# ifpen/wfcrl-env

Hardware: AMD Instinct MI355X
Metric: farm_steps_per_sec (higher is better)
Workload: dtype f32

## Files before the change

include/wfstep.h:

```cpp
#ifndef WFSTEP_H
#define WFSTEP_H

#ifdef __cplusplus
extern "C" {
#endif

#define WF_ABI_VERSION 7

#define WF_OK 0
#define WF_E_INVALID -1
#define WF_E_UNSUPPORTED -2
#define WF_E_NODEVICE -3
#define WF_E_HIP -4
#define WF_E_NOMEM -5

#define WF_MAX_TURBINES 256
#define WF_MAX_TABLE 64
#define WF_MAX_TURBINE_TYPES 4

typedef struct wf_handle wf_handle;

typedef struct wf_model_params {
  double air_density, ambient_ti, shear, veer;
  double rotor_diameter, hub_height, tsr, pP, pT, gen_eff, ref_density;
// ... 40 lines not shown
int wf_set_layouts_counts(wf_handle* h, int n_layouts, const double* x, const double* y, const int* counts, const int* layout_of);

int wf_set_wind(wf_handle* h, const double* ws, const double* wd, int count, int on_device);

int wf_set_wind_counts(wf_handle* h, const double* ws, int n_ws, const double* wd, int n_wd, int on_device);

int wf_step(wf_handle* h, const float* yaw, float* power, float* wind_speed, float* wind_dir, float* load,
            int on_device);

int wf_sync(wf_handle* h);

#define WF_RISK_OVERLAP 1
#define WF_RISK_POWER_KNEE 2
#define WF_RISK_THRUST_RAMP 4
#define WF_RISK_THRUST_UNITY 8
#define WF_RISK_NEGATIVE_SPEED 16
int wf_set_risk_guard(wf_handle* h, double rel_band);
int wf_get_risk_flags(wf_handle* h, int* flags, int on_device);

int wf_set_risk_resolve(wf_handle* h, int mode);
int wf_get_risk_resolve(wf_handle* h, int* mode);
int wf_get_resolve_stats(wf_handle* h, int* n_resolved, int* raw_flags, int on_device);

typedef struct wf_env_params {
  float yaw_lo, yaw_hi, yaw_step;
  float actuator_rate;
  float dt;
  float budget;
  float load_coef;
  int discrete;
} wf_env_params;

int wf_env_config(wf_handle* h, const wf_env_params* p);

int wf_env_set_power_unit(wf_handle* h, int megawatts);

int wf_env_reset(wf_handle* h);

int wf_env_step(wf_handle* h, const float* action, float* reward, float* yaw, float* power, float* wind_speed,
                float* wind_dir, float* load, int on_device);

int wf_env_set_prev_wind(wf_handle* h, const double* wind_speed , int on_device);

int wf_env_state(wf_handle* h, float* yaw, float* acc, int* moves, int set, int on_device);

typedef struct wf_wind_dist {
// ... 49 lines not shown
```

wfcrl-env_amd/_lib.py:

```python
from __future__ import annotations

import ctypes as C
import os
import subprocess
from pathlib import Path

PKG_DIR = Path(__file__).resolve().parent
LIB_PATH = PKG_DIR / "libwfstep.so"

WF_OK = 0
WF_RISK_OVERLAP = 1
WF_RISK_POWER_KNEE = 2
WF_RISK_THRUST_RAMP = 4
WF_RISK_THRUST_UNITY = 8
WF_RISK_NEGATIVE_SPEED = 16
WF_E = {-1: "WF_E_INVALID", -2: "WF_E_UNSUPPORTED", -3: "WF_E_NODEVICE", -4: "WF_E_HIP", -5: "WF_E_NOMEM"}

_MODEL_DOUBLES = (
    "air_density", "ambient_ti", "shear", "veer",
    "rotor_diameter", "hub_height", "tsr", "pP", "pT", "gen_eff", "ref_density",
    "alpha", "beta", "ka", "kb", "ad", "bd", "dm",
    "ch_initial", "ch_constant", "ch_ai", "ch_downstream",
    "eps_gain", "num_eps", "kappa", "gch_gain", "overlap_thresh", "near_wake_c",
    "defl_alpha", "defl_beta", "defl_ka", "defl_kb",
# ... 46 lines not shown
    "wf_turbine_table": (C.c_int, [C.c_char_p, C.POINTER(C.c_int), C.POINTER(C.POINTER(C.c_double)),
                                   C.POINTER(C.POINTER(C.c_double)), C.POINTER(C.POINTER(C.c_double))]),
    "wf_create": (C.c_int, [C.c_int, C.POINTER(_P)]),
    "wf_destroy": (C.c_int, [_P]),
    "wf_set_stream": (C.c_int, [_P, _P, C.c_int]),
    "wf_get_stream": (_P, [_P]),
    "wf_set_model": (C.c_int, [_P, C.POINTER(ModelParams)]),
    "wf_set_turbine_types": (C.c_int, [_P, C.c_int, C.POINTER(TurbineDef), C.POINTER(C.c_int)]),
    "wf_get_turbine_types": (C.c_int, [_P, C.POINTER(C.c_int)]),
    "wf_set_layout": (C.c_int, [_P, C.c_int, _P, _P]),
    "wf_set_batch": (C.c_int, [_P, C.c_int]),
    "wf_set_layouts": (C.c_int, [_P, C.c_int, _P, _P, _P]),
    "wf_set_layouts_counts": (C.c_int, [_P, C.c_int, _P, _P, _P, _P]),
    "wf_set_wind": (C.c_int, [_P, _P, _P, C.c_int, C.c_int]),
    "wf_set_wind_counts": (C.c_int, [_P, _P, C.c_int, _P, C.c_int, C.c_int]),
    "wf_wind_sample_binned": (C.c_int, [_P, C.c_ulonglong, C.POINTER(WindDist), C.c_double]),
    "wf_step": (C.c_int, [_P, _P, _P, _P, _P, _P, C.c_int]),
    "wf_sync": (C.c_int, [_P]),
    "wf_set_risk_guard": (C.c_int, [_P, C.c_double]),
    "wf_get_risk_flags": (C.c_int, [_P, _P, C.c_int]),
    "wf_set_risk_resolve": (C.c_int, [_P, C.c_int]),
    "wf_get_risk_resolve": (C.c_int, [_P, C.POINTER(C.c_int)]),
    "wf_get_resolve_stats": (C.c_int, [_P, C.POINTER(C.c_int), _P, C.c_int]),
    "wf_wind_sample": (C.c_int, [_P, C.c_ulonglong, C.POINTER(WindDist)]),
    "wf_wind_series": (C.c_int, [_P, C.c_int, _P, _P, _P, C.c_ulonglong]),
    "wf_wind_series_step": (C.c_int, [_P]),
    "wf_get_wind": (C.c_int, [_P, _P, _P, C.c_int]),
    "wf_env_config": (C.c_int, [_P, C.POINTER(EnvParams)]),
    "wf_env_set_power_unit": (C.c_int, [_P, C.c_int]),
    "wf_env_reset": (C.c_int, [_P]),
    "wf_env_state": (C.c_int, [_P, _P, _P, _P, C.c_int, C.c_int]),
    "wf_env_set_prev_wind": (C.c_int, [_P, _P, C.c_int]),
    "wf_env_step": (C.c_int, [_P, _P, _P, _P, _P, _P, _P, _P, C.c_int]),
    "wf_timing_begin": (C.c_int, [_P]),
    "wf_timing_end": (C.c_int, [_P, C.POINTER(C.c_float)]),
    "wf_get_kernel_info": (C.c_int, [_P, C.POINTER(KernelInfo)]),
    "wf_set_kernel_choice": (C.c_int, [_P, C.POINTER(KernelChoice)]),
    "wf_get_kernel_choice": (C.c_int, [_P, C.POINTER(KernelChoice)]),
    "wf_get_calibration": (C.c_int, [_P, C.POINTER(C.c_int), C.POINTER(C.c_float)]),
    "wf_get_fly_calibration": (C.c_int, [_P, C.POINTER(C.c_int), C.POINTER(C.c_float)]),
    "wf_get_mixed_launch": (C.c_int, [_P, C.POINTER(C.c_int), C.POINTER(C.c_float)]),
    "wf_calibrate": (C.c_int, [_P]),
    "wf_set_calibration": (C.c_int, [_P, C.c_int, C.c_int]),
    "wf_last_error": (C.c_char_p, [_P]),
}

# ... 50 lines not shown
```

wfcrl-env_amd/backend.py:

```python
from __future__ import annotations

import ctypes as C

import numpy as np

from . import _lib
from ._lib import EnvParams, KernelChoice, KernelInfo, ModelParams, WindDist, check


def _is_torch(a) -> bool:
    return type(a).__module__.startswith("torch")


def default_model() -> dict:
    p = ModelParams()
    check(_lib.load().wf_default_model(C.byref(p)))
    d = {n: getattr(p, n) for n in _lib._MODEL_DOUBLES}
    d.update({n: bool(getattr(p, n)) for n in _lib._MODEL_SWITCHES})
    n = p.n_table
    d["table_ws"] = [p.table_ws[i] for i in range(n)]
    d["table_ct"] = [p.table_ct[i] for i in range(n)]
    d["table_cp"] = [p.table_cp[i] for i in range(n)]
    return d

# ... 301 lines not shown
                    out[k] = torch.empty(shapes[k], device=dev, dtype=torch.float32)
            ptrs = [out[k].data_ptr() if k in want else None for k in order]
            check(self._lib.wf_env_step(self._h, action.data_ptr() if action is not None else None, *ptrs, 1), self._h)
            return {k: out[k] for k in want}
        if action is not None:
            action = np.ascontiguousarray(action, dtype=np.float32).reshape(B, N)
        out = dict(out or {})
        for k in want:
            if k not in out:
                out[k] = np.empty(shapes[k], np.float32)
        ptrs = [out[k].ctypes.data if k in want else None for k in order]
        check(self._lib.wf_env_step(self._h, action.ctypes.data if action is not None else None, *ptrs, 0), self._h)
        return {k: out[k] for k in want}

    def sync(self):
        check(self._lib.wf_sync(self._h), self._h)

    def set_risk_guard(self, rel_band: float):
        check(self._lib.wf_set_risk_guard(self._h, float(rel_band)), self._h)

    def set_risk_resolve(self, mode: int | bool = 1):
        check(self._lib.wf_set_risk_resolve(self._h, int(mode)), self._h)

    def risk_resolve(self) -> int:
        m = C.c_int(0)
        check(self._lib.wf_get_risk_resolve(self._h, C.byref(m)), self._h)
        return int(m.value)

    def resolve_stats(self) -> dict:
        if not self.risk_resolve():
            raise RuntimeError("resolve_stats() needs the float64 re-solve on (set_risk_resolve(1), the default); with it off "
                               "the flags of the last step are risk_flags()")
        n = C.c_int(0)
        raw = np.empty(self.env_batch, np.int32)
        check(self._lib.wf_get_resolve_stats(self._h, C.byref(n), raw.ctypes.data, 0), self._h)
        return {"n_resolved": int(n.value), "raw_flags": raw}

    def risk_flags(self, as_torch: bool = False):
        B = self.env_batch
        if as_torch:
            import torch

            self._follow_torch_stream()
            f = torch.empty(B, dtype=torch.int32, device=f"cuda:{self.device_id}")
            check(self._lib.wf_get_risk_flags(self._h, f.data_ptr(), 1), self._h)
            return f
# ... 90 lines not shown
```

wfcrl-env_amd/csrc/wf_abi.hip:

```cpp
#include "wf_handle.h"

namespace wfi {

thread_local std::string g_create_error;

void free_batch(wf_handle* h) {
  hipFree(h->d_ws); hipFree(h->d_wd); hipFree(h->d_gx); hipFree(h->d_gy); hipFree(h->d_gidx); hipFree(h->d_flags);
  hipFree(h->d_farm_tie);
  hipFree(h->d_dir_perm); hipFree(h->d_sort_keys); hipFree(h->d_sort_vals); hipFree(h->d_sort_tmp);
  h->d_dir_perm = h->d_sort_vals = nullptr; h->d_sort_keys = nullptr; h->d_sort_tmp = nullptr;
  h->sort_tmp_bytes = h->dir_perm_cap = 0; h->dir_slots = 0;
  hipFree(h->d_res_list); hipFree(h->d_res_count); hipFree(h->d_flags_raw);
  h->d_res_list = h->d_res_count = h->d_flags_raw = nullptr;
  if (h->h_res_seen) (void)hipHostFree(h->h_res_seen);
  h->h_res_seen = nullptr;
  h->d_flags = h->d_farm_tie = nullptr;
  hipFree(h->d_yaw); hipFree(h->d_out);
  hipFree(h->d_env_yaw); hipFree(h->d_env_acc); hipFree(h->d_env_act); hipFree(h->d_env_out); hipFree(h->d_env_moves);
  if (h->h_env_act) hipHostFree(h->h_env_act);
  if (h->h_env_out) hipHostFree(h->h_env_out);
  h->d_env_yaw = h->d_env_acc = h->d_env_act = h->d_env_out = h->h_env_act = h->h_env_out = nullptr;
  h->d_env_moves = nullptr;
  hipFree(h->d_series_ws); hipFree(h->d_series_wd); hipFree(h->d_series_start); hipFree(h->d_ws_prev);
  hipFree(h->d_pair_tab); hipFree(h->d_pair_first); h->d_pair_tab = nullptr; h->d_pair_first = nullptr; h->pair_dirty = true;
// ... 257 lines not shown
  if (wspd) std::memcpy(wspd, h->h_out + bn, sizeof(float) * bn);
  if (wdir) std::memcpy(wdir, h->h_out + 2 * bn, sizeof(float) * bn);
  if (load) std::memcpy(load, h->h_out + 3 * bn, sizeof(float) * bn * 4);
  return WF_OK;
}
int wf_set_risk_guard(wf_handle* h, double rel_band) {
  if (!h) return WF_E_INVALID;
  if (!(rel_band >= 0.0) || !(rel_band < 0.5)) return fail(h, WF_E_INVALID, "risk guard band must be in [0, 0.5)");
  h->guard_rel = rel_band;
  h->guard_user = true;
  h->consts.guard_inv = rel_band > 0.0 ? (float)(1.0 / rel_band) : 1125899906842624.0f;
  return WF_OK;
}

int wf_set_risk_resolve(wf_handle* h, int mode) {
  if (!h) return WF_E_INVALID;
  if (mode < 0 || mode > 2) return fail(h, WF_E_INVALID, "risk resolve mode must be 0 (off), 1 (flagged farms) or 2 (every farm)");
  if (!h->types.empty() && mode == 0)
    return fail(h, WF_E_INVALID, "several turbine definitions (wf_set_turbine_types): the float32 kernels know one table, mode 0 cannot be served");
  h->resolve_mode = mode;
  return WF_OK;
}

int wf_get_risk_resolve(wf_handle* h, int* mode) {
  if (!h || !mode) return WF_E_INVALID;
  *mode = h->types.empty() ? h->resolve_mode : 2;
  return WF_OK;
}

int wf_get_resolve_stats(wf_handle* h, int* n_resolved, int* raw_flags, int on_device) {
  if (!h) return WF_E_INVALID;
  if (h->B <= 0) return fail(h, WF_E_INVALID, "wf_set_batch must be called first");
  WF_ON_DEVICE(h);
  if (!h->d_res_list || !h->res_last) {
    if (n_resolved) *n_resolved = 0;
    if (raw_flags) return wf_get_risk_flags(h, raw_flags, on_device);
    return WF_OK;
  }
  if (raw_flags)
    WF_HIP(h, hipMemcpyAsync(raw_flags, h->d_flags_raw, sizeof(int) * h->B, on_device ? hipMemcpyDeviceToDevice : hipMemcpyDeviceToHost,
                             h->stream));
  if (n_resolved) WF_HIP(h, hipMemcpyAsync(n_resolved, h->d_res_count + h->res_parity, sizeof(int), hipMemcpyDeviceToHost, h->stream));
  if (n_resolved || (raw_flags && !on_device)) WF_HIP(h, hipStreamSynchronize(h->stream));
  return WF_OK;
}

// ... 36 lines not shown
```

wfcrl-env_amd/csrc/wf_device.h:

```cpp
#pragma once

#define WF_TABLE_PAD 64
#define WF_BUCKETS 2048

struct WfConsts {
  int N;
  float D, invD;
  float off[3];
  float yoff[3];
  float shearf[3];
  float uinf_f;
  float decay_a[3];
  float exp_c;
  float zc[7], zc2[7], ez[7];
  float inv_eps2, m_half_inv_eps4, yl2_small;
  float zm[7], zm2[7], ezm[7];
  int mirror_core_n;
  float gam_top, gam_bot;
  float gam_wr;
  float ks_top, ks_bot, ks_core;
  float alpha4, beta2, ka, kb, ad, bd, dm03;
  float alpha4_d, beta2_d, ka_d, kb_d;
  float sw_steer, sw_tv;
  float e0c1, e0c2;
  float sz0v;
  float near_c;
  float kdef;
  float kdef_sy0v;
  float far_k;
  int far_on;
  float ch_c, ch_ai, ch_down;
  float amb, amb2, gch_gain, overlap_thr, twoD;
  float rho, pw, dens_f;
  int n_table;
  float bucket_h_inv, bucket_x0;
  int max_probe;
  double fifteenD_d;
  double q_d;
  float ct_kappa;
  float guard_inv, inv_overlap_thr, knee_kappa;
  int veer_on;
  float cos_veer;
  float veer_c2, veer_s2;
  float veer_bq;
};

struct WfTables {
  float knot[WF_TABLE_PAD];
  float ct[WF_TABLE_PAD];
  float ct_slope[WF_TABLE_PAD];
  float pw[WF_TABLE_PAD];
  float pw_slope[WF_TABLE_PAD];
  unsigned char bucket[WF_BUCKETS];
// ... 78 lines not shown
```

wfcrl-env_amd/csrc/wf_handle.h:

```cpp
#pragma once
#include <hip/hip_runtime.h>

#include <cmath>
#include <cstdio>
#include <cstdlib>
#include <cstring>
#include <mutex>
#include <new>
#include <string>
#include <vector>

#include "../../include/wfstep.h"
#include "wf_device.h"
#include "wf_resolve.h"

extern "C" hipError_t wfk_launch_resolve(const WfResolveConsts* c, const WfResolveArgs* a, int B, int all, int* raw_flags,
                                         int n_cu, hipStream_t s);
extern "C" int wfk_num_variants();
extern "C" void wfk_variant(int i, int* G, int* S, const void** fn);
extern "C" int wfk_variant_has_table(int i);
extern "C" int wfk_tab_waves();
extern "C" const void* wfk_variant_fn(int i, int kind);
extern "C" hipError_t wfk_launch_geometry(int n_env, int N, const double* lx, const double* ly, const double* centre,
                                          int layout_mode, const int* layout_of, const int* layout_n, const double* wd, int wd_stride, double* gx,
// ... 104 lines not shown
  int* d_ll_flag = nullptr;
  float* d_src_log = nullptr;
  size_t ll_groups_cap = 0, log_records_cap = 0;
  int* d_farm_tie = nullptr;
  int* d_dir_perm = nullptr;
  float* d_sort_keys = nullptr;
  int* d_sort_vals = nullptr;
  void* d_sort_tmp = nullptr;
  size_t sort_tmp_bytes = 0, dir_perm_cap = 0;
  int dir_slots = 0;
  int geo_tie_block = 0;
  int farm_ties = 2;
  bool wind_sync = true;
  int ll_ties = 2;
  wf_kernel_choice choice{0, 0, -1, 0, 0, -1, -1, -1, -1, -1};
  int n_cu = 256;
  bool calib_done = false;
  int calib_code = -1;
  int mix_main = 0;
  bool tab_slot = false;
  float calib_ms[8] = {};
  int fly_calib = 0;
  float fly_calib_ms[2] = {};
  int resolve_mode = 1;
  WfResolveConsts rconsts{};
  double* d_tab64 = nullptr;
  int *d_res_list = nullptr, *d_res_count = nullptr, *d_flags_raw = nullptr;
  int* h_res_seen = nullptr;
  int res_parity = 0;
  bool res_last = false;
  int res_mask = 0;
  struct TurbineType {
    std::vector<double> ws, ct, cp;
    double tsr, pP, gen_eff, ref_density;
  };
  std::vector<TurbineType> types;
  std::vector<int> type_of;
  double* d_tab64_mt = nullptr;
  double* d_type_consts = nullptr;
  int* d_type_of = nullptr;
};

namespace wfi {

extern thread_local std::string g_create_error;

// ... 58 lines not shown
```

wfcrl-env_amd/csrc/wf_kernels_ll.hip:

```cpp
#include <hip/hip_runtime.h>

#include <cstring>
#include <type_traits>
#include <utility>

#include "wf_kernel_common.h"

namespace {

template <class F, int... I>
__device__ __forceinline__ void static_for_impl(F&& f, std::integer_sequence<int, I...>) {
  (f(std::integral_constant<int, I>{}), ...);
}
template <int N, class F>
__device__ __forceinline__ void static_for(F&& f) {
  static_for_impl(f, std::make_integer_sequence<int, N>{});
}

__device__ __forceinline__ void sincos_yaw(float x, float& s, float& c) {
  const float x2 = x * x;
  s = x * fmaf(x2, fmaf(x2, fmaf(x2, fmaf(x2, 2.7557319e-6f, -1.9841270e-4f), 8.3333333e-3f), -1.6666667e-1f), 1.0f);
  c = fmaf(x2, fmaf(x2, fmaf(x2, fmaf(x2, fmaf(x2, -2.7557319e-7f, 2.4801587e-5f), -1.3888889e-3f), 4.1666667e-2f), -0.5f), 1.0f);
  if (__any(fabsf(x) > 0.8f)) {
    float s2, c2;
// ... 440 lines not shown
    const float ti = fabsf(R.ch_pref) * tipow;
    const float tia = in15 ? ti * (cnt * (1.0f / 9.0f)) : 0.0f;
    const float cand = fsqrt(fmaf(tia, tia, c.amb2));
#pragma unroll
    for (int j = 0; j < 3; ++j) {
      const float cm = (bits & (1 << j)) ? cand : 0.0f;
      TI[p][j] = __uint_as_float(max(__float_as_uint(TI[p][j]), __float_as_uint(cm)));
    }
  };

  float psum = 0.0f, lsum = 0.0f;
  const int n_real = ga.n_real ? ga.n_real[env] : N;
#ifdef WF_LL_STAMP
  unsigned long long st_acc[12] = {0, 0, 0, 0, 0, 0, 0, 0, 0, 0, 0, 0};
  WF_T(st_begin);
#endif
  int q = 0;
  const size_t wave_rec0 = (size_t)(slot - eiw) * n_pad;
  float2* const log_hot = reinterpret_cast<float2*>(src_log + wave_rec0 * WF_LOG_HOT_FLOATS);
  float4* const log_cold = reinterpret_cast<float4*>(src_log + log_cold_offset + wave_rec0 * WF_LOG_COLD_FLOATS) + eiw;
  float4* const bndL = reinterpret_cast<float4*>(yaw_lds) + (size_t)wave * n_pad;
  constexpr int HOT_INSTR = (CH / 2) * EPW * 16 >= 1024 ? (CH / 2) * EPW * 16 / 1024 : 1;
  constexpr int HOT_F4 = HOT_INSTR * 64;
  float4* const hotL = reinterpret_cast<float4*>(yaw_lds) + (size_t)WPB * n_pad + (size_t)wave * (2 * HOT_F4);
  auto stage_hot = [&](int qq, int i_first) {
    const char* g0 = reinterpret_cast<const char*>(reinterpret_cast<const float4*>(log_hot) + (size_t)(i_first >> 1) * EPW);
    char* l0 = reinterpret_cast<char*>(hotL + (qq & 1) * HOT_F4);
#pragma unroll
    for (int ch = 0; ch < HOT_INSTR; ++ch) lds_dma16(g0 + ch * 1024 + lane * 16, l0 + ch * 1024, true);
  };
  auto hot_index = [&](int i) { return 2 * ((size_t)(i >> 1) * EPW + eiw) + (i & 1); };
  auto load_hot = [&](int i) { return log_hot[hot_index(i)]; };
  auto load_cold = [&](int i) {
    const float4* lp = log_cold + (size_t)i * (3 * EPW);
    ColdRec r;
    r.a = lp[0]; r.b = lp[EPW]; r.c = lp[2 * EPW];
    return r;
  };
  const float snw_f = c.near_c * 0.70710678118f;
  auto unpack = [&](const float2 h, const ColdRec& r) {
    SrcLog R;
    R.Gy = h.x * h.y; R.Gwt = h.y;
    R.sy0d = r.a.x; R.sz0d = r.a.y; R.sM = r.a.z; R.tan_th0 = r.a.w;
    R.sy0v = r.b.x; R.x0d = r.b.y; R.kyd = r.b.z; R.pj = r.b.w;
    R.x0v = r.c.x; R.kyv = r.c.y; R.ch_pref = r.c.z; R.ix0v = r.c.w;
    R.snw = snw_f * R.sM;
    R.kdef = (R.sM * R.sM) * (R.sy0v * c.kdef_sy0v);
// ... 42 lines not shown
    const int n_src = min(N, first_own + GS);
    const int n_chunks = (n_src + CH - 1) / CH;
    float2 hot_nx = make_float2(0.0f, 0.0f);
    ColdRec cold_nx = {};
    double xs_nx = 0.0, ys_nx = 0.0;
    if (first_own > 0) {
      if constexpr (!TAB) {
        hot_nx = load_hot(0);
        cold_nx = load_cold(0);
        xs_nx = gx[gofs];
        ys_nx = gy[gofs];
      }
    }

    auto fly_record = [&](auto PP, double xi, double yi) {
      constexpr int p = decltype(PP)::value;
      constexpr int q = TAB ? 0 : p;
      float4 r;
      r.x = (float)(xt_d[q] - xi);
      r.y = (float)(yt_d[q] - yi);
      r.z = (xt_d[q] <= xi + c.fifteenD_d) ? 1.0f : 0.0f;
      r.w = __int_as_float((xt_d[q] > xi + 0.1) ? 8 : 0);
      return r;
    };

    auto own_source = [&](auto PS, int i, const float* recs) {
      constexpr int ps = decltype(PS)::value;
      const int src = gbase + ((i - first_own) - ps * G);
      __builtin_amdgcn_s_setprio(3);
      WF_T(so_0);
      float vsum = 0.0f;
#pragma unroll
      for (int k2 = 0; k2 < 9; ++k2) vsum += V[ps][k2];
      const float m3 = __shfl(cube_sum(esq[ps]), src);
      const float Vmean = __shfl(vsum, src) * (1.0f / 9.0f);
      float TIs[3];
#pragma unroll
      for (int j = 0; j < 3; ++j) TIs[j] = __shfl(TI[ps][j], src);
      const float yaw_i = __shfl(yaw_t[ps], src);
      const float cg = __shfl(cg_t[ps], src), sg = __shfl(sg_t[ps], src);
      WF_T(so_1);
      WF_ACC(6, so_0, so_1);
      SrcLog Sc;
      const float ubar = fcbrt_pos(m3 * (1.0f / 9.0f));
      unsigned trisk;
      const float ct = table_ct(c, T, ubar, trisk) * cg;
// ... 79 lines not shown
      if (lane == src) {
#pragma unroll
        for (int j = 0; j < 3; ++j) TI[ps][j] = fmaxf(TI[ps][j] + X.dTI, amb0);
      }
      Sc.sy0v = c.sz0v * cg;
      if constexpr (VEER) Sc.sy0v *= c.cos_veer;
      Sc.snw = c.near_c * fsqrt(0.5f * ct);
      Sc.kdef = ct * cg * c.kdef;
      Sc.ch_pref = c.ch_c * fexp2(c.ch_ai * flog2(a));
      const float x0num_v = c.D * cg * (1.0f + s_c) * (1.0f / 1.41421356237f);
      const float b2om = c.beta2 * om_sc, b2om_d = c.beta2_d * om_sc;
      Sc.x0d = x0num_d * frcp(fmaf(c.alpha4_d, TIs[0], b2om_d));
      Sc.kyd = fmaf(c.ka_d, TIs[0], c.kb_d);
      Sc.pj = pfac * frcp(Sc.kyd);
      Sc.x0v = x0num_v * frcp(fmaf(c.alpha4, TIs[0] + X.dTI, b2om));
      Sc.kyv = fmaf(c.ka, TIs[0] + X.dTI, c.kb);
      X.TI0 = TIs[0]; X.TI1 = TIs[1]; X.TI2 = TIs[2];
      const bool split = !((TIs[0] == TIs[1]) && (TIs[1] == TIs[2]));
      Sc.ch_pref = split ? -Sc.ch_pref : Sc.ch_pref;
      Sc.ix0v = frcp(Sc.x0v);
      Sc.inv_s0d = frcp(Sc.sy0d * Sc.sz0d);
      Sc.d0 = Sc.tan_th0 * Sc.x0d;
      if (J + 1 < nblk) {
        if (sub == 0) {
          log_hot[hot_index(i)] = make_float2(Sc.Gwt != 0.0f ? Sc.Gy * frcp(Sc.Gwt) : 0.0f, Sc.Gwt);
          float4* lp = log_cold + (size_t)i * (3 * EPW);
          lp[0] = make_float4(Sc.sy0d, Sc.sz0d, Sc.sM, Sc.tan_th0);
          lp[EPW] = make_float4(Sc.sy0v, Sc.x0d, Sc.kyd, Sc.pj);
          lp[2 * EPW] = make_float4(Sc.x0v, Sc.kyv, Sc.ch_pref, Sc.ix0v);
          if (split) *reinterpret_cast<float4*>(logx + (size_t)i * WF_LOG_SIDE_FLOATS) = make_float4(X.TI0, X.TI1, X.TI2, X.dTI);
        }
        const float s0 = VEER ? c.sz0v : Sc.sy0v;
        float kyv_m = Sc.kyv, bb = fmaf(-Sc.kyv, Sc.x0v, s0);
        float db = fabsf(Sc.tan_th0 * Sc.x0d) + 2.2f * fabsf(Sc.pj);
        if (__any(split)) {
          const float TImax = fmaxf(TIs[0], fmaxf(TIs[1], TIs[2])), TImin = fminf(TIs[0], fminf(TIs[1], TIs[2]));
          const float x0d_m = x0num_d * frcp(fmaf(c.alpha4_d, TImin, b2om_d));
          const float pj_m = pfac * frcp(fmaf(c.ka_d, TImin, c.kb_d));
          kyv_m = fmaf(c.ka, TImax + X.dTI, c.kb);
          bb = split ? s0 : bb;
          db = fabsf(Sc.tan_th0 * x0d_m) + 2.2f * fabsf(pj_m);
        }
        const float dbo = db + c.off[2];
        float k6 = c.far_k * kyv_m, b6 = fmaf(c.far_k, bb, dbo), n6 = fmaf(c.far_k, fmaxf(Sc.snw, s0), dbo);
        k6 = wave_max<G>(k6);
        b6 = wave_max<G>(b6);
        n6 = wave_max<G>(n6);
        if (!c.far_on) { k6 = 0.0f; b6 = 0.0f; n6 = 3.0e38f; }
        if (lane == 0) bndL[i] = make_float4(k6, b6, n6, 0.0f);
      }
      WF_T(so_4);
      WF_ACC(9, so_3, so_4);
      const float xs_[4] = {X.TI0, X.TI1, X.TI2, X.dTI};
      static_for<S>([&](auto PP) {
        constexpr int p = decltype(PP)::value;
        if constexpr (p == ps) pass2(PP, Sc, xs_, false, ex[p], ex[p].x > 0.0f, yt_d[TAB ? 0 : p], yi_d);
        else if constexpr (p > ps) pass2(PP, Sc, xs_, false, ex[p], tvalid[p], yt_d[TAB ? 0 : p], yi_d);
      });
      WF_T(so_5);
      WF_ACC(10, so_4, so_5);
      __builtin_amdgcn_s_setprio(0);
    };

    for (int cq = 0; cq < n_chunks; ++cq, ++q) {
      if constexpr (TAB) {
        if (cq == 0 && first_own > 0) wf_dma_wait();
        if (cq + 1 < n_chunks || J + 1 < nblk) stage_chunk(q + 1);
        if (cq + 1 < n_chunks && (cq + 1) * CH < first_own) stage_hot(q + 1, (cq + 1) * CH);
      }
      const float* buf = &prow[q & 1][0];
      const int i0 = cq * CH;
      const int k_log = min(max(first_own - i0, 0), CH);
      const int k_end = min(n_src - i0, CH);
      WF_T(st_a);
      auto within_bound = [&](const float4 bnd, float dx, float dy) {
        return fabsf(dy) < fmaxf(fmaf(bnd.x, dx, bnd.y), bnd.z) + fabsf(fmaf(c.bd, dx, c.ad));
      };
      if constexpr (TAB) {
        if (k_log > 0) {
          unsigned long long near_bits, pair_bits;
          {
            const int kk = lane / GS, rr = lane % GS;
            const float2 e = *reinterpret_cast<const float2*>(buf + (kk * GS + rr) * WF_PAIR_STRIDE + WF_PAIR_DX);
            const float4 bnd = bndL[min(i0 + kk, n_pad - 1)];
            pair_bits = __ballot(kk < k_log && (J * GS + rr) < N && within_bound(bnd, e.x, e.y));
            near_bits = pair_bits;
#pragma unroll
            for (int sh = 1; sh < GS; sh <<= 1) near_bits |= near_bits >> sh;
            unsigned long long rep = 0ull;
#pragma unroll
            for (int kq = 0; kq < CH; ++kq) rep |= 1ull << (kq * GS);
            near_bits &= rep;
          }
          ColdRec cold_nx = {};
          if (near_bits) cold_nx = load_cold(i0 + (__builtin_ctzll(near_bits) / GS));
          static_assert(GS % 2 == 0 && CH % 2 == 0, "logged sources come in pairs");
#pragma unroll 1
          for (int k = 0; k < k_log; k += 2) {
            const float4 hot2 = hotL[(q & 1) * HOT_F4 + (k >> 1) * EPW + eiw];
            float4 cf[S][9];
// ... 57 lines not shown
          hot_nx = load_hot(inx);
          cold_nx = load_cold(inx);
          xs_nx = gx[gofs + inx];
          ys_nx = gy[gofs + inx];
          const float4 bnd = bndL[i];
          float4 exr[S];
          int nr = 0;
          static_for<S>([&](auto PP) {
            constexpr int p = decltype(PP)::value;
            exr[p] = fly_record(PP, xs_d, ys_d);
            nr |= (int)tvalid[p] & (int)within_bound(bnd, exr[p].x, exr[p].y);
          });
          const bool near = __any(nr != 0);
          const SrcLog Sl = unpack(hot, cold);
          static_for<S>([&](auto PP) {
            constexpr int p = decltype(PP)::value;
            if (tvalid[p]) apply_fly(PP, exr[p].x, exr[p].y, hot.x * hot.y, hot.y);
            if (near) pass2(PP, Sl, side, true, exr[p], tvalid[p], yt_d[TAB ? 0 : p], ys_d);
          });
        }
      }
      WF_T(st_b);
      WF_ACC(0, st_a, st_b);
#pragma unroll 1
      for (int k = k_log; k < k_end; ++k) {
        const int i = i0 + k;
        const float* recs = buf + (k * GS) * WF_PAIR_STRIDE;
        const int slot_of_source = (i - first_own) / G;
        static_for<S>([&](auto PS) {
          if (slot_of_source == decltype(PS)::value) own_source(PS, i, recs);
        });
      }
      WF_T(st_c);
      WF_ACC(1, st_b, st_c);
      if constexpr (TAB) {
        wf_dma_wait();
        __syncthreads();
      }
      WF_T(st_d);
      WF_ACC(2, st_c, st_d);
    }
    if constexpr (TAB) {
      if (J + 1 < nblk) stage_hot(q, 0);
    }
    WF_T(st_e);

#pragma unroll
    for (int p = 0; p < S; ++p) {
// ... 98 lines not shown
      const float r = psum * invN * 1.0e-3f * frcp(wr * wr * wr) - ea.load_coef * lsum * invN * 0.25f;
      ea.reward[env] = r;
    }
  }
}

constexpr int kLLWaves = 4;

template <int G, int S, bool TAB, bool MC1, bool VEER = false>
static hipError_t launch_ll(const WfConsts* c, const WfTables* tab, const int* gidx, const double* ws, const double* wd,
                            int wind_stride, const float* yaw, float* power, float* o_ws, float* o_wd, float* load, int B,
                            const WfEnvArgs* env, const float* ll_tab, const int* cross_tie, float* src_log, size_t log_records,
                            const WfGroupArgs* grp, const double* gx, const double* gy, hipStream_t s) {
  constexpr int fpb = kLLWaves * (64 / G);
  WfGroupArgs ga = *grp;
  const int n_farms = ga.env_end ? ga.env_end - ga.env_base : B;
  const int grid = ga.blk_group ? (ga.n_slots + fpb - 1) / fpb : (n_farms + fpb - 1) / fpb;
  WfConsts cc = *c;
  WfEnvArgs ea;
  if (env) ea = *env; else memset(&ea, 0, sizeof(ea));
  size_t group_floats = wfk_ll_table_floats(cc.N, G * S);
  int n_pad = ((cc.N + G * S - 1) / (G * S)) * (G * S);
  constexpr int hot_bytes = 32768 / (G * G * S) >= 1024 ? 32768 / (G * G * S) : 1024;
  const size_t dyn_lds = sizeof(float4) * (size_t)kLLWaves * n_pad + (TAB ? (size_t)kLLWaves * 2 * hot_bytes : 0);
  size_t log_cold_offset = log_records * WF_LOG_HOT_FLOATS, log_side_offset = log_records * WF_LOG_FLOATS;
  void* args[] = {&cc, &tab, &gidx, &ws, &wd, &wind_stride, &yaw, &power, &o_ws, &o_wd, &load, &B, &ea, &ll_tab,
                  &group_floats, &cross_tie, &src_log, &log_cold_offset, &log_side_offset, &n_pad, &ga, &gx, &gy};
  const void* fn = (const void*)&wf_step_ll_kernel<G, S, false, TAB, MC1, kLLWaves, VEER>;
  if constexpr (TAB) {
    if (wind_stride == 0) fn = (const void*)&wf_step_ll_kernel<G, S, true, TAB, MC1, kLLWaves, VEER>;
  }
  if constexpr (S == 1 && (MC1 || !TAB) && !VEER) {
    static int n_cu_of[64] = {};
    int dev = 0, n_cu = 0;
    if (hipGetDevice(&dev) == hipSuccess && dev >= 0 && dev < 64) {
      n_cu = n_cu_of[dev];
      if (n_cu == 0 && hipDeviceGetAttribute(&n_cu, hipDeviceAttributeMultiprocessorCount, dev) == hipSuccess) n_cu_of[dev] = n_cu;
    }
    if (n_cu > 0 && grid <= 2 * n_cu)
      fn = wind_stride == 0 ? (const void*)&wf_step_ll_kernel<G, S, true, TAB, MC1, kLLWaves, VEER, true>
                            : (const void*)&wf_step_ll_kernel<G, S, false, TAB, MC1, kLLWaves, VEER, true>;
  }
  return hipLaunchKernel(fn, dim3(grid), dim3(64 * kLLWaves), args, dyn_lds, s);
}

extern "C" int wfk_ll_farms_per_block(int G) { return kLLWaves * (64 / G); }
#ifdef WF_LL_STAMP
// ... 98 lines not shown
```

wfcrl-env_amd/csrc/wf_model.hip:

```cpp
#include "wf_handle.h"

namespace {

const double kCtFrom3[45] = {
    0.99,       0.99,       0.97373036, 0.92826162, 0.89210543, 0.86100905, 0.835423,   0.81237673, 0.79225789,
    0.77584769, 0.7629228,  0.76156073, 0.76261984, 0.76169723, 0.75232027, 0.74026851, 0.72987175, 0.70701647,
    0.54054532, 0.45509459, 0.39343381, 0.34250785, 0.30487242, 0.27164979, 0.24361964, 0.21973831, 0.19918151,
    0.18131868, 0.16537679, 0.15103727, 0.13998636, 0.1289037,  0.11970413, 0.11087113, 0.10339901, 0.09617888,
    0.09009926, 0.08395078, 0.0791188,  0.07448356, 0.07050731, 0.06684119, 0.06345518, 0.06032267, 0.05741999};
const double kCpFrom3SurveyA5[45] = {
    0.1780851,  0.28907459, 0.34902166, 0.3847278,  0.40605878, 0.4202279,  0.42882274, 0.43387274, 0.43622267,
    0.43684468, 0.43657497, 0.43651053, 0.4365612,  0.43651728, 0.43590309, 0.43467276, 0.43322955, 0.43003137,
    0.37655587, 0.33328466, 0.29700574, 0.26420779, 0.23839379, 0.21459275, 0.19382354, 0.1756635,  0.15970926,
    0.14561785, 0.13287856, 0.12130194, 0.11219941, 0.10311631, 0.09545392, 0.08813781, 0.08186763, 0.07585005,
    0.07071926, 0.06557558, 0.06148104, 0.05755207, 0.05413366, 0.05097969, 0.04806545, 0.04536883, 0.04287006};
const double kCpFrom3Floris3[45] = {
    0.178085, 0.289075, 0.349022, 0.384728, 0.406059, 0.420228, 0.428823, 0.433873, 0.436223,
    0.436845, 0.436575, 0.436511, 0.436561, 0.436517, 0.435903, 0.434673, 0.433230, 0.430466,
    0.378869, 0.335199, 0.297991, 0.266092, 0.238588, 0.214748, 0.193981, 0.175808, 0.159835,
    0.145741, 0.133256, 0.122157, 0.112257, 0.103399, 0.095449, 0.088294, 0.081836, 0.075993,
    0.070692, 0.065875, 0.061484, 0.057476, 0.053809, 0.050447, 0.047358, 0.044518, 0.041900,
};
double g_tab_ws[51], g_tab_ct[51], g_tab_cp[51], g_tab_cp_a5[51];
std::once_flag g_tab_once;
// ... 74 lines not shown
  c.gam_bot = (float)(inv2pi * (M_PI / 8.0) * D * vel_bot * uinf);
  c.gam_wr = (float)(inv2pi * 0.25 * 2.0 * M_PI * D / m.tsr);
  c.alpha4 = (float)(4.0 * m.alpha); c.beta2 = (float)(2.0 * m.beta);
  c.ka = (float)m.ka; c.kb = (float)m.kb; c.ad = (float)m.ad; c.bd = (float)m.bd; c.dm03 = (float)(0.3 * m.dm);
  c.alpha4_d = (float)(4.0 * m.defl_alpha); c.beta2_d = (float)(2.0 * m.defl_beta);
  c.ka_d = (float)m.defl_ka; c.kb_d = (float)m.defl_kb;
  c.sw_steer = m.enable_secondary_steering ? 2.0f : 0.0f;
  c.sw_tv = m.enable_transverse_velocities ? 1.0f : 0.0f;
  c.e0c1 = (float)(3.0 * std::exp(1.0 / 12.0)); c.e0c2 = (float)(3.0 * std::exp(1.0 / 3.0));
  c.sz0v = (float)(D / (2.0 * std::sqrt(2.0)));
  c.near_c = (float)(m.near_wake_c * D);
  c.kdef = (float)(D * D / 8.0);
  c.ch_c = (float)(m.ch_constant * std::pow(m.ambient_ti, m.ch_initial));
  c.ch_ai = (float)m.ch_ai; c.ch_down = (float)m.ch_downstream;
  c.amb = (float)m.ambient_ti; c.amb2 = (float)(m.ambient_ti * m.ambient_ti);
  c.gch_gain = m.enable_yaw_added_recovery ? (float)m.gch_gain : 0.0f; c.overlap_thr = (float)m.overlap_thresh;
  c.twoD = (float)(2.0 * D); c.fifteenD_d = 15.0 * D;
  c.q_d = D / 4.0;
  c.guard_inv = h->guard_rel > 0.0 ? (float)(1.0 / h->guard_rel) : 1125899906842624.0f;
  c.inv_overlap_thr = (float)(1.0 / m.overlap_thresh);
  c.far_on = (h->choice.far_skip != 0 && m.ka >= 0.0 && m.kb >= 0.0 && m.defl_ka >= 0.0 && m.defl_kb >= 0.0 && m.alpha >= 0.0 &&
              m.beta >= 0.0 && m.defl_alpha >= 0.0 && m.defl_beta >= 0.0) ? 1 : 0;
  c.far_k = c.far_on ? 6.12f : 1.0e30f;
  c.ct_kappa = 5.0f;
  c.knee_kappa = 30.0f;
  {
    const double vr = m.veer * M_PI / 180.0;
    c.veer_on = m.veer != 0.0 ? 1 : 0;
    c.cos_veer = (float)std::cos(vr);
    c.veer_c2 = (float)(std::cos(vr) * std::cos(vr)); c.veer_s2 = (float)(std::sin(vr) * std::sin(vr));
    c.veer_bq = (float)(std::sin(2.0 * vr) * D / 4.0);
    c.kdef_sy0v = (float)((D * D / 8.0) / ((D / (2.0 * std::sqrt(2.0))) * std::cos(vr)));
  }
  c.rho = (float)m.ref_density; c.pw = (float)(m.pP / 3.0);
  c.dens_f = (float)std::cbrt(m.air_density / m.ref_density);

  WfTables t;
  const double area = M_PI * R * R;
  std::vector<double> pwv(n);
  for (int i = 0; i < n; ++i) pwv[i] = 0.5 * area * h->tcp[i] * m.gen_eff * h->tws[i] * h->tws[i] * h->tws[i];
  for (int i = 0; i < WF_TABLE_PAD; ++i) {
    const bool in = i < n;
    t.knot[i] = in ? (float)h->tws[i] : 3.0e38f;
    t.ct[i] = in ? (float)h->tct[i] : 0.f;
    t.pw[i] = in ? (float)pwv[i] : 0.f;
    const bool seg = i + 1 < n;
// ... 233 lines not shown
```

Measured before the change: 81.92 million.

## Solve independent wake sources as a parallel level with snapshot rollback

Adds a speculative 'level' path to the low-latency kernel: all owned sources in a chunk are processed together, with one parallel velocity accumulation and parameter computation, instead of the sequential per-source loop. The current state is snapshotted into LDS first. A ballot-based bound check then verifies that no owned source affects another. If the check fails, the state is restored and the sequential loop runs. This is meant to cut the serial dependency chain for farms whose sources do not interact, at the cost of extra LDS for the snapshot, possibly lower occupancy (guarded by an LDS-fit check), and wasted work when the check fails. A new ABI setter controls the mode, and it defaults to on.

Result: faster. 84.76 million, median of 6 (+3.5%).

```diff
diff --git a/include/wfstep.h b/include/wfstep.h
--- a/include/wfstep.h
+++ b/include/wfstep.h
@@ -86,6 +86,8 @@
 int wf_get_risk_resolve(wf_handle* h, int* mode);
 int wf_get_resolve_stats(wf_handle* h, int* n_resolved, int* raw_flags, int on_device);
 
+int wf_set_ll_levels(wf_handle* h, int mode);
+
 typedef struct wf_env_params {
   float yaw_lo, yaw_hi, yaw_step;
   float actuator_rate;
diff --git a/wfcrl-env_amd/_lib.py b/wfcrl-env_amd/_lib.py
--- a/wfcrl-env_amd/_lib.py
+++ b/wfcrl-env_amd/_lib.py
@@ -92,6 +92,7 @@
     "wf_set_risk_resolve": (C.c_int, [_P, C.c_int]),
     "wf_get_risk_resolve": (C.c_int, [_P, C.POINTER(C.c_int)]),
     "wf_get_resolve_stats": (C.c_int, [_P, C.POINTER(C.c_int), _P, C.c_int]),
+    "wf_set_ll_levels": (C.c_int, [_P, C.c_int]),
     "wf_wind_sample": (C.c_int, [_P, C.c_ulonglong, C.POINTER(WindDist)]),
     "wf_wind_series": (C.c_int, [_P, C.c_int, _P, _P, _P, C.c_ulonglong]),
     "wf_wind_series_step": (C.c_int, [_P]),
diff --git a/wfcrl-env_amd/backend.py b/wfcrl-env_amd/backend.py
--- a/wfcrl-env_amd/backend.py
+++ b/wfcrl-env_amd/backend.py
@@ -347,6 +347,9 @@
     def set_risk_resolve(self, mode: int | bool = 1):
         check(self._lib.wf_set_risk_resolve(self._h, int(mode)), self._h)
 
+    def set_ll_levels(self, mode: int = 1):
+        check(self._lib.wf_set_ll_levels(self._h, int(mode)), self._h)
+
     def risk_resolve(self) -> int:
         m = C.c_int(0)
         check(self._lib.wf_get_risk_resolve(self._h, C.byref(m)), self._h)
diff --git a/wfcrl-env_amd/csrc/wf_abi.hip b/wfcrl-env_amd/csrc/wf_abi.hip
--- a/wfcrl-env_amd/csrc/wf_abi.hip
+++ b/wfcrl-env_amd/csrc/wf_abi.hip
@@ -303,6 +303,14 @@
   return WF_OK;
 }
 
+int wf_set_ll_levels(wf_handle* h, int mode) {
+  if (!h) return WF_E_INVALID;
+  if (mode < 0 || mode > 2) return fail(h, WF_E_INVALID, "level mode must be 0 (off), 1 (on) or 2 (on, every level check failed)");
+  h->ll_levels = mode;
+  h->consts.ll_levels = mode;
+  return WF_OK;
+}
+
 int wf_get_risk_resolve(wf_handle* h, int* mode) {
   if (!h || !mode) return WF_E_INVALID;
   *mode = h->types.empty() ? h->resolve_mode : 2;
diff --git a/wfcrl-env_amd/csrc/wf_device.h b/wfcrl-env_amd/csrc/wf_device.h
--- a/wfcrl-env_amd/csrc/wf_device.h
+++ b/wfcrl-env_amd/csrc/wf_device.h
@@ -29,6 +29,7 @@
   float kdef_sy0v;
   float far_k;
   int far_on;
+  int ll_levels;
   float ch_c, ch_ai, ch_down;
   float amb, amb2, gch_gain, overlap_thr, twoD;
   float rho, pw, dens_f;
diff --git a/wfcrl-env_amd/csrc/wf_handle.h b/wfcrl-env_amd/csrc/wf_handle.h
--- a/wfcrl-env_amd/csrc/wf_handle.h
+++ b/wfcrl-env_amd/csrc/wf_handle.h
@@ -150,6 +150,7 @@
   float calib_ms[8] = {};
   int fly_calib = 0;
   float fly_calib_ms[2] = {};
+  int ll_levels = 1;
   int resolve_mode = 1;
   WfResolveConsts rconsts{};
   double* d_tab64 = nullptr;
diff --git a/wfcrl-env_amd/csrc/wf_kernels_ll.hip b/wfcrl-env_amd/csrc/wf_kernels_ll.hip
--- a/wfcrl-env_amd/csrc/wf_kernels_ll.hip
+++ b/wfcrl-env_amd/csrc/wf_kernels_ll.hip
@@ -486,7 +486,11 @@
   float4* const bndL = reinterpret_cast<float4*>(yaw_lds) + (size_t)wave * n_pad;
   constexpr int HOT_INSTR = (CH / 2) * EPW * 16 >= 1024 ? (CH / 2) * EPW * 16 / 1024 : 1;
   constexpr int HOT_F4 = HOT_INSTR * 64;
-  float4* const hotL = reinterpret_cast<float4*>(yaw_lds) + (size_t)WPB * n_pad + (size_t)wave * (2 * HOT_F4);
+  constexpr bool LVL_LDS = TAB && !VEER && S == 2;
+  constexpr bool LVL = LVL_LDS && UWS;
+  constexpr int SNAP_F4 = LVL_LDS ? (18 * S + 3) / 4 * 64 : 0;
+  const int hot_stride = (LVL_LDS && c.ll_levels != 0 && SNAP_F4 > 2 * HOT_F4) ? SNAP_F4 : 2 * HOT_F4;
+  float4* const hotL = reinterpret_cast<float4*>(yaw_lds) + (size_t)WPB * n_pad + (size_t)wave * hot_stride;
   auto stage_hot = [&](int qq, int i_first) {
     const char* g0 = reinterpret_cast<const char*>(reinterpret_cast<const float4*>(log_hot) + (size_t)(i_first >> 1) * EPW);
     char* l0 = reinterpret_cast<char*>(hotL + (qq & 1) * HOT_F4);
@@ -575,6 +579,10 @@
       r.z = (xt_d[q] <= xi + c.fifteenD_d) ? 1.0f : 0.0f;
       r.w = __int_as_float((xt_d[q] > xi + 0.1) ? 8 : 0);
       return r;
+    };
+
+    auto within_bound = [&](const float4 bnd, float dx, float dy) {
+      return fabsf(dy) < fmaxf(fmaf(bnd.x, dx, bnd.y), bnd.z) + fabsf(fmaf(c.bd, dx, c.ad));
     };
 
     auto own_source = [&](auto PS, int i, const float* recs) {
@@ -700,7 +708,7 @@
       Sc.inv_s0d = frcp(Sc.sy0d * Sc.sz0d);
       Sc.d0 = Sc.tan_th0 * Sc.x0d;
       if (J + 1 < nblk) {
-        if (sub == 0) {
+        if (LVL ? lane == src : sub == 0) {
           log_hot[hot_index(i)] = make_float2(Sc.Gwt != 0.0f ? Sc.Gy * frcp(Sc.Gwt) : 0.0f, Sc.Gwt);
           float4* lp = log_cold + (size_t)i * (3 * EPW);
           lp[0] = make_float4(Sc.sy0d, Sc.sz0d, Sc.sM, Sc.tan_th0);
@@ -740,6 +748,217 @@
       __builtin_amdgcn_s_setprio(0);
     };
 
+    auto own_level = [&](auto k0, int nm, const float* recs0) {
+      __builtin_amdgcn_s_setprio(3);
+      WF_T(lv_0);
+      constexpr int NSF = (18 * S + 3) / 4 * 4;
+      auto snap_f = [&](int f) -> float& { return f % 18 < 9 ? V[f / 18][f % 18] : W[f / 18][f % 18 - 9]; };
+      {
+        float x[NSF];
+#pragma unroll
+        for (int f = 0; f < NSF; ++f) x[f] = f < 18 * S ? snap_f(f) : 0.0f;
+#pragma unroll
+        for (int c4 = 0; c4 < NSF / 4; ++c4) hotL[c4 * 64 + lane] = make_float4(x[4 * c4], x[4 * c4 + 1], x[4 * c4 + 2], x[4 * c4 + 3]);
+      }
+      float ubar_l[S], ct_l[S], a_l[S], Gwr_l[S], Gy_l[S], Gwt_l[S];
+      unsigned trisk_l[S];
+      WF_T(lv_1);
+      WF_ACC(6, lv_0, lv_1);
+#pragma unroll
+      for (int p = 0; p < S; ++p) {
+        const float m3 = cube_sum(esq[p]);
+        const float cg = cg_t[p], sg = sg_t[p];
+        const float ubar = fcbrt_pos(m3 * (1.0f / 9.0f));
+        const float ct = table_ct(c, T, ubar, trisk_l[p]) * cg;
+        const float sq1 = fsqrt(1.0f - ct * cg);
+        const float a = 0.5f * ct * frcp(1.0f + sq1);
+        const float Gwr = c.gam_wr * (a - a * a) * ubar;
+        const float scg = sg * cg * c.sw_tv;
+        ubar_l[p] = ubar; ct_l[p] = ct; a_l[p] = a; Gwr_l[p] = Gwr;
+        Gy_l[p] = scg * ct * ws;
+        Gwt_l[p] = Gwr * c.sw_tv;
+      }
+      WF_T(lv_2);
+      WF_ACC(7, lv_1, lv_2);
+      float vm_l[S], vb_l[S], wb_l[S];
+      static_for<S>([&](auto PS) {
+        constexpr int ps = decltype(PS)::value;
+        vm_l[ps] = 0.0f; vb_l[ps] = 0.0f; wb_l[ps] = 0.0f;
+#pragma unroll 1
+        for (int s = 0; s < G; ++s) {
+          const int m = ps * G + s;
+          if (m >= nm) break;
+          const int src = gbase + s;
+          float vsum = 0.0f;
+#pragma unroll
+          for (int k2 = 0; k2 < 9; ++k2) vsum += V[ps][k2];
+          vm_l[ps] = (sub == s) ? vsum : vm_l[ps];
+          const float Gy = __shfl(Gy_l[ps], src), Gwt = __shfl(Gwt_l[ps], src);
+          const float* recs = recs0 + ((k0 + m) * GS) * WF_PAIR_STRIDE;
+          static_for<S>([&](auto PP) {
+            constexpr int p = decltype(PP)::value;
+            const float* rec = recs + (p * G + sub) * WF_PAIR_STRIDE;
+            const bool act1 = (p > ps) ? tvalid[p] : (rec[WF_PAIR_DX] >= 0.0f);
+            if (p >= ps || __any(act1)) {
+              if (act1) apply_tab(PP, reinterpret_cast<const float4*>(rec), Gy, Gwt);
+            }
+            __builtin_amdgcn_sched_barrier(0);
+          });
+          float vbar = 0.0f, wbar = 0.0f;
+#pragma unroll
+          for (int k2 = 0; k2 < 9; ++k2) { vbar += V[ps][k2]; wbar += W[ps][k2]; }
+          vb_l[ps] = (sub == s) ? vbar : vb_l[ps];
+          wb_l[ps] = (sub == s) ? wbar : wb_l[ps];
+        }
+      });
+      WF_T(lv_3);
+      WF_ACC(8, lv_2, lv_3);
+      float dTI_l[S] = {};
+      constexpr unsigned long long farms = ~0ull / ((1ull << G) - 1ull);
+      auto pick = [](const auto& x, int p) {
+        auto r = x[0];
+#pragma unroll
+        for (int q = 1; q < S; ++q) r = (p == q) ? x[q] : r;
+        return r;
+      };
+#pragma unroll 1
+      for (int p = 0; p < S; ++p) {
+        const int i = first_own + p * G + sub;
+        const float cg = pick(cg_t, p), sg = pick(sg_t, p), yaw_i = pick(yaw_t, p);
+        const float ct = pick(ct_l, p), ubar = pick(ubar_l, p), a = pick(a_l, p), Gwr = pick(Gwr_l, p);
+        const float Vmean = pick(vm_l, p) * (1.0f / 9.0f);
+        const float vbar = pick(vb_l, p) * (1.0f / 9.0f), wbar = pick(wb_l, p) * (1.0f / 9.0f);
+        const bool tv = pick(tvalid, p);
+        float TIs[3];
+#pragma unroll
+        for (int j = 0; j < 3; ++j) {
+          TIs[j] = TI[0][j];
+#pragma unroll
+          for (int q = 1; q < S; ++q) TIs[j] = (p == q) ? TI[q][j] : TIs[j];
+        }
+        const float gt = c.gam_top * ws * ct, gb = c.gam_bot * ws * ct;
+        SrcLog Sc;
+        Sc.Gy = pick(Gy_l, p); Sc.Gwt = pick(Gwt_l, p);
+        float val = c.sw_steer * (Vmean - Gwr * c.ks_core) * frcp(gt * c.ks_top - gb * c.ks_bot);
+        val = fminf(fmaxf(val, -1.0f), 1.0f);
+        float asv = asin_small(val);
+        if (((__ballot(fabsf(val) > 0.3f) >> sub) & farms) != 0ull) asv = asinf(val);
+        const float gd = -(yaw_i * kDeg2Rad + 0.5f * asv);
+        const float c2h = fsqrt(fmaxf(fmaf(-val, val, 1.0f), 0.0f));
+        const float chh = fsqrt(0.5f * (1.0f + c2h));
+        const float shh = 0.5f * val * frcp(chh);
+        const float cgd = fmaf(cg, chh, -sg * shh);
+        const float s_cc = fsqrt(1.0f - ct * cgd), s_c = fsqrt(1.0f - ct);
+        const float om_scc = ct * cgd * frcp(1.0f + s_cc);
+        const float om_sc = ct * frcp(1.0f + s_c);
+        Sc.sM = fsqrt(ct);
+        const float E0 = fmaf(om_sc, om_sc, fmaf(-c.e0c1, om_sc, c.e0c2));
+        Sc.sz0d = 0.5f * c.D * fsqrt((1.0f + s_cc) * frcp(2.0f * (1.0f + s_c)));
+        Sc.sy0d = Sc.sz0d * cgd;
+        const float th0 = c.dm03 * gd * frcp(cgd) * om_scc;
+        {
+          const float t2 = th0 * th0;
+          const float poly = th0 * fmaf(t2, fmaf(t2, fmaf(t2, fmaf(t2, fmaf(t2, 0.0088632355f, 0.0218694885f), 0.0539682540f),
+                                                            0.1333333333f), 0.3333333333f), 1.0f);
+          Sc.tan_th0 = poly;
+          if (__any(fabsf(th0) > 0.35f)) {
+            const float rev = th0 * 0.15915494309189535f;
+            const float hw = __builtin_amdgcn_sinf(rev) * frcp(__builtin_amdgcn_cosf(rev));
+            Sc.tan_th0 = (fabsf(th0) > 0.35f) ? hw : poly;
+          }
+        }
+        const float pfac = th0 * E0 * (1.0f / 5.2f) * fsqrt(Sc.sy0d * Sc.sz0d * frcp(ct)) * kLn2;
+        const float x0num_d = c.D * cgd * (1.0f + s_cc) * (1.0f / 1.41421356237f);
+        const float I0 = TIs[0];
+        const float uI = ubar * I0;
+        const float mix2 = (vbar * vbar + wbar * wbar) * (1.0f / 3.0f);
+        const float inv_ubar = frcp(ubar);
+        const float Itot = fsqrt(fmaf(uI, uI, mix2)) * inv_ubar;
+        const float Imix = mix2 * inv_ubar * inv_ubar * frcp(Itot + I0);
+        const float dTI = c.gch_gain * Imix;
+#pragma unroll
+        for (int q = 0; q < S; ++q) dTI_l[q] = (p == q) ? dTI : dTI_l[q];
+        Sc.sy0v = c.sz0v * cg;
+        Sc.snw = c.near_c * fsqrt(0.5f * ct);
+        Sc.ch_pref = c.ch_c * fexp2(c.ch_ai * flog2(a));
+        const float x0num_v = c.D * cg * (1.0f + s_c) * (1.0f / 1.41421356237f);
+        const float b2om = c.beta2 * om_sc, b2om_d = c.beta2_d * om_sc;
+        Sc.x0d = x0num_d * frcp(fmaf(c.alpha4_d, TIs[0], b2om_d));
+        Sc.kyd = fmaf(c.ka_d, TIs[0], c.kb_d);
+        Sc.pj = pfac * frcp(Sc.kyd);
+        Sc.x0v = x0num_v * frcp(fmaf(c.alpha4, TIs[0] + dTI, b2om));
+        Sc.kyv = fmaf(c.ka, TIs[0] + dTI, c.kb);
+        const bool split = !((TIs[0] == TIs[1]) && (TIs[1] == TIs[2]));
+        Sc.ch_pref = split ? -Sc.ch_pref : Sc.ch_pref;
+        Sc.ix0v = frcp(Sc.x0v);
+        if (J + 1 < nblk && tv) {
+          log_hot[hot_index(i)] = make_float2(Sc.Gwt != 0.0f ? Sc.Gy * frcp(Sc.Gwt) : 0.0f, Sc.Gwt);
+          float4* lp = log_cold + (size_t)i * (3 * EPW);
+          lp[0] = make_float4(Sc.sy0d, Sc.sz0d, Sc.sM, Sc.tan_th0);
+          lp[EPW] = make_float4(Sc.sy0v, Sc.x0d, Sc.kyd, Sc.pj);
+          lp[2 * EPW] = make_float4(Sc.x0v, Sc.kyv, Sc.ch_pref, Sc.ix0v);
+          if (split) *reinterpret_cast<float4*>(logx + (size_t)i * WF_LOG_SIDE_FLOATS) = make_float4(TIs[0], TIs[1], TIs[2], dTI);
+        }
+        const float s0 = Sc.sy0v;
+        float kyv_m = Sc.kyv, bb = fmaf(-Sc.kyv, Sc.x0v, s0);
+        float db = fabsf(Sc.tan_th0 * Sc.x0d) + 2.2f * fabsf(Sc.pj);
+        if (__any(split)) {
+          const float TImax = fmaxf(TIs[0], fmaxf(TIs[1], TIs[2])), TImin = fminf(TIs[0], fminf(TIs[1], TIs[2]));
+          const float x0d_m = x0num_d * frcp(fmaf(c.alpha4_d, TImin, b2om_d));
+          const float pj_m = pfac * frcp(fmaf(c.ka_d, TImin, c.kb_d));
+          kyv_m = fmaf(c.ka, TImax + dTI, c.kb);
+          bb = split ? s0 : bb;
+          db = fabsf(Sc.tan_th0 * x0d_m) + 2.2f * fabsf(pj_m);
+        }
+        const float dbo = db + c.off[2];
+        float k6 = c.far_k * kyv_m, b6 = fmaf(c.far_k, bb, dbo), n6 = fmaf(c.far_k, fmaxf(Sc.snw, s0), dbo);
+#pragma unroll
+        for (int w = G; w < 64; w <<= 1) {
+          k6 = fmaxf(k6, __shfl_xor(k6, w));
+          b6 = fmaxf(b6, __shfl_xor(b6, w));
+          n6 = fmaxf(n6, __shfl_xor(n6, w));
+        }
+        if (!c.far_on) { k6 = 0.0f; b6 = 0.0f; n6 = 3.0e38f; }
+        if (lane < G) bndL[i] = make_float4(k6, b6, n6, 0.0f);
+      }
+      WF_T(lv_4);
+      WF_ACC(9, lv_3, lv_4);
+      unsigned long long fails = 0ull;
+#pragma unroll
+      for (int a0 = 0; a0 < GS; a0 += 64 / GS) {
+        const int am = a0 + lane / GS, bm = lane % GS;
+        const float4 e = *reinterpret_cast<const float4*>(recs0 + ((k0 + am) * GS + bm) * WF_PAIR_STRIDE + WF_PAIR_DX);
+        const float4 bnd = bndL[first_own + am];
+        fails |= __ballot(am < bm && bm < nm &&
+                          (within_bound(bnd, e.x, e.y) || (e.z > 0.0f && (__float_as_int(e.w) & 7) != 0)));
+      }
+      const bool ok = c.ll_levels != 2 && fails == 0ull;
+      if (ok) {
+        unsigned tr = 0u;
+#pragma unroll
+        for (int p = 0; p < S; ++p) {
+          if (!tvalid[p]) continue;
+          tr |= trisk_l[p];
+#pragma unroll
+          for (int j = 0; j < 3; ++j) TI[p][j] = fmaxf(TI[p][j] + dTI_l[p], amb0);
+        }
+        if (tr) atomicOr(&risk_lds[wave][eiw], tr);
+      } else {
+#pragma unroll
+        for (int c4 = 0; c4 < NSF / 4; ++c4) {
+          const float4 v4 = hotL[c4 * 64 + lane];
+          const float x[4] = {v4.x, v4.y, v4.z, v4.w};
+#pragma unroll
+          for (int e = 0; e < 4; ++e)
+            if (4 * c4 + e < 18 * S) snap_f(4 * c4 + e) = x[e];
+        }
+      }
+      WF_T(lv_5);
+      WF_ACC(10, lv_4, lv_5);
+      __builtin_amdgcn_s_setprio(0);
+      return ok;
+    };
+
     for (int cq = 0; cq < n_chunks; ++cq, ++q) {
       if constexpr (TAB) {
         if (cq == 0 && first_own > 0) wf_dma_wait();
@@ -751,9 +970,6 @@
       const int k_log = min(max(first_own - i0, 0), CH);
       const int k_end = min(n_src - i0, CH);
       WF_T(st_a);
-      auto within_bound = [&](const float4 bnd, float dx, float dy) {
-        return fabsf(dy) < fmaxf(fmaf(bnd.x, dx, bnd.y), bnd.z) + fabsf(fmaf(c.bd, dx, c.ad));
-      };
       if constexpr (TAB) {
         if (k_log > 0) {
           unsigned long long near_bits, pair_bits;
@@ -857,8 +1073,12 @@
       }
       WF_T(st_b);
       WF_ACC(0, st_a, st_b);
+      bool solved = false;
+      if constexpr (LVL) {
+        if (c.ll_levels != 0 && k_end > k_log) solved = own_level(k_log, k_end - k_log, buf);
+      }
 #pragma unroll 1
-      for (int k = k_log; k < k_end; ++k) {
+      for (int k = solved ? k_end : k_log; k < k_end; ++k) {
         const int i = i0 + k;
         const float* recs = buf + (k * GS) * WF_PAIR_STRIDE;
         const int slot_of_source = (i - first_own) / G;
@@ -1003,7 +1223,17 @@
   size_t group_floats = wfk_ll_table_floats(cc.N, G * S);
   int n_pad = ((cc.N + G * S - 1) / (G * S)) * (G * S);
   constexpr int hot_bytes = 32768 / (G * G * S) >= 1024 ? 32768 / (G * G * S) : 1024;
-  const size_t dyn_lds = sizeof(float4) * (size_t)kLLWaves * n_pad + (TAB ? (size_t)kLLWaves * 2 * hot_bytes : 0);
+  constexpr bool lvl_lds = TAB && !VEER && S == 2;
+  constexpr int snap_bytes = lvl_lds ? (18 * S + 3) / 4 * 64 * 16 : 0;
+  size_t hot_stride = 2 * (size_t)hot_bytes;
+  if (lvl_lds && cc.ll_levels != 0 && snap_bytes > 2 * hot_bytes) {
+    const size_t lds_cu = 163840, stat = sizeof(TableLds) + 2 * 64 * WF_PAIR_STRIDE * 4 + 2 * kLLWaves * (64 / G) * 4 + 256;
+    const size_t bnd = sizeof(float4) * (size_t)kLLWaves * n_pad;
+    const size_t with = stat + bnd + (size_t)kLLWaves * snap_bytes, without = stat + bnd + (size_t)kLLWaves * hot_stride;
+    if (std::min<size_t>(2, lds_cu / with) >= std::min<size_t>(2, lds_cu / without)) hot_stride = snap_bytes;
+    else cc.ll_levels = 0;
+  }
+  const size_t dyn_lds = sizeof(float4) * (size_t)kLLWaves * n_pad + (TAB ? (size_t)kLLWaves * hot_stride : 0);
   size_t log_cold_offset = log_records * WF_LOG_HOT_FLOATS, log_side_offset = log_records * WF_LOG_FLOATS;
   void* args[] = {&cc, &tab, &gidx, &ws, &wd, &wind_stride, &yaw, &power, &o_ws, &o_wd, &load, &B, &ea, &ll_tab,
                   &group_floats, &cross_tie, &src_log, &log_cold_offset, &log_side_offset, &n_pad, &ga, &gx, &gy};
diff --git a/wfcrl-env_amd/csrc/wf_model.hip b/wfcrl-env_amd/csrc/wf_model.hip
--- a/wfcrl-env_amd/csrc/wf_model.hip
+++ b/wfcrl-env_amd/csrc/wf_model.hip
@@ -120,6 +120,7 @@
   c.far_on = (h->choice.far_skip != 0 && m.ka >= 0.0 && m.kb >= 0.0 && m.defl_ka >= 0.0 && m.defl_kb >= 0.0 && m.alpha >= 0.0 &&
               m.beta >= 0.0 && m.defl_alpha >= 0.0 && m.defl_beta >= 0.0) ? 1 : 0;
   c.far_k = c.far_on ? 6.12f : 1.0e30f;
+  c.ll_levels = h->ll_levels;
   c.ct_kappa = 5.0f;
   c.knee_kappa = 30.0f;
   {
```
